# Priceincoding/nebula

Hardware: AMD Instinct MI355X
Metric: GTEPS for GO 3 STEPS on RMAT-26 at 1/2/4/8 GPUs; % of HBM roofline (higher is better)
Workload: dtype int64; 1 GPU; GO 3 STEPS FROM 64 seeds OVER follow WHERE follow.weight > 499 YIELD DISTINCT follow._dst; RMAT-26 ef16; vertices=32803048, edges_after_collapse=1060378721, edges_scanned_per_query=1545132647, parallelism=1 GPU

## Files before the change

### nebula_amd/csrc/bottom_up.hip

```cpp
#include <algorithm>
#include <cstdio>
#include <cstdlib>
#include <mutex>
#include <string>
#include <unordered_map>
#include <vector>

#include "device_common.h"
#include "engine.h"
#include "expr_device.h"
#include "go_device.h"
#include "go_launch.h"
#include "qpred.h"
#include "query_common.h"

namespace nbg {

__global__ __launch_bounds__(1024) void k_reduce_partials(const unsigned long long* partials, int nblocks,
                                                          unsigned long long* out,
                                                          const unsigned long long* gate = nullptr) {
  if (gate && *gate == 0ull) return;
  __shared__ unsigned long long s[kSlots][16];
  unsigned long long a[kSlots];
#pragma unroll
// ... 89 lines not shown
#pragma unroll
      for (int j = 0; j < R; j++) {
        const int64_t bj = __shfl((long long)rb[j], my_src), ej = __shfl((long long)re[j], my_src);
        if (my_j == j) {
          b = bj;
          e = ej;
        }
      }
      acc[3] += gl == 0 && my_j >= 0;
      bool f = false;
      for (int64_t x = b;; x += GL * ru) {
        const bool act = !f && x < e;
        if (__ballot(act) == 0) break;
        bool h = false;
        if (act) {
          int32_t sr[kRestMax];
#pragma unroll
          for (int u = 0; u < kRestMax; u++) {
            const int64_t ex = x + u * GL + gl;
            sr[u] = (u < ru && ex < e) ? tcol[ex] : -1;
          }
#pragma unroll
          for (int u = 0; u < kRestMax; u++) {
            const int64_t ex = x + u * GL + gl;
            if (sr[u] < 0) continue;
            acc[4]++;
            if (entry(sr[u], ex)) h = true;
          }
        }
        const unsigned long long hb = __ballot(h);
        if (act && ((hb >> (grp * GL)) & ((1ull << GL) - 1ull))) f = true;
      }
#pragma unroll
      for (int g = 0; g < NG; g++) {
        const int sj = __shfl(my_j, g * GL), ss = __shfl(my_src, g * GL);
        const int fg = __shfl(int(f), g * GL);
#pragma unroll
        for (int j = 0; j < R; j++)
          if (sj == j && lane == ss) found[j] = fg != 0;
      }
    }
  }
}

template <int PK, int U, int HUB, int STATS, int NT = 0, int SKIP = 0>
__global__ __launch_bounds__(1024, 8) void k_bu_lean(const uint2* __restrict__ lo, const uint2* __restrict__ hi,
                                                     int64_t ntiles, int64_t work_tiles,
                                                     const uint32_t* __restrict__ fbits, uint32_t fb_bytes,
                                                     unsigned long long* __restrict__ nbits,
                                                     unsigned long long* __restrict__ pbits,
                                                     const uint32_t* __restrict__ odeg, QArgs q_arg,
                                                     unsigned long long* __restrict__ partials, int cw,
                                                     const uint8_t* __restrict__ odeg8,
                                                     unsigned long long* gate, GateIn gi, int atomic_sums) {
  if (!gate_open(gi, gate)) return;
  __shared__ unsigned long long lds[kSlots * 16];
  extern __shared__ uint32_t s_fb[];
  if (HUB) hub_fill(s_fb, fbits, cw, true);
  const QArgs q = q_sgpr(q_arg);
  constexpr bool FINAL = PK == PK_FAST;
  constexpr int NS = FINAL ? 4 : 2;
  const __amdgpu_buffer_rsrc_t fb_rs =
      __builtin_amdgcn_make_buffer_rsrc(const_cast<uint32_t*>(fbits), 0, int(fb_bytes), 0x00020000);
  const uint32_t gmask = q.gmask, ucw = uint32_t(cw);
  const int lane = threadIdx.x & 63;
  const int64_t wave = (int64_t(blockIdx.x) * blockDim.x + threadIdx.x) >> 6;
  const int64_t nwaves = (int64_t(gridDim.x) * blockDim.x) >> 6;
  uint32_t nglob = 0, nhub = 0;
  unsigned long long nfound = 0, npend = 0, nwords = 0;
  unsigned long long odsum = 0;
  auto prep = [&](uint32_t sw, int k, uint32_t& goff, uint32_t& lidx, uint32_t& pm, uint32_t& um) {
    const uint32_t wi = (sw & gmask) >> 5;
    bool cand = true;
    if (FINAL) {
      const int st = q_test(int32_t(sw), q);
      const bool und = st < 0, pass = st > 0;
      cand = st != 0;
      pm |= pass ? 1u << k : 0u;
      um |= und ? 1u << k : 0u;
    }
    const bool hub = HUB && wi < ucw;
    goff = cand && !hub ? wi * 4u : 0xfffffff0u;
    lidx = cand && hub ? wi : ucw;
    if (STATS) {
      nglob += cand && !hub;
      nhub += cand && hub;
    }
  };
  auto bit = [](uint32_t w, uint32_t sw) -> uint32_t { return __builtin_amdgcn_ubfe(w, sw & 31u, 1u); };
  auto row_of = [&](int64_t t, int h) -> int64_t { return t * 128 + lane + 64 * h; };
  for (int64_t t0 = wave * U; t0 < work_tiles; t0 += nwaves * U) {
    uint2 a[U][2], b[U][2];
    uint32_t od[U][2];
    bool v[U];
#pragma unroll
    for (int u = 0; u < U; u++) {
      v[u] = t0 + u < work_tiles;
      const int64_t r = (v[u] ? t0 + u : t0) * 128 + lane;
#pragma unroll
      for (int h = 0; h < 2; h++) {
        if (NT) {
          const uint64_t x = __builtin_nontemporal_load(reinterpret_cast<const uint64_t*>(lo + r + 64 * h));
          a[u][h] = make_uint2(uint32_t(x), uint32_t(x >> 32));
          if (FINAL) {
            const uint64_t y = __builtin_nontemporal_load(reinterpret_cast<const uint64_t*>(hi + r + 64 * h));
            b[u][h] = make_uint2(uint32_t(y), uint32_t(y >> 32));
          }
          od[u][h] = FINAL ? 1u : uint32_t(__builtin_nontemporal_load(odeg8 + r + 64 * h));
        } else {
          a[u][h] = lo[r + 64 * h];
          if (FINAL) b[u][h] = hi[r + 64 * h];
          od[u][h] = FINAL ? 1u : odeg[r + 64 * h];
        }
      }
    }
    __builtin_amdgcn_sched_barrier(0);
    uint32_t goff[U][2][NS], lidx[U][2][NS], pm[U][2], um[U][2];
#pragma unroll
    for (int u = 0; u < U; u++)
#pragma unroll
      for (int h = 0; h < 2; h++) {
        pm[u][h] = um[u][h] = 0u;
        prep(a[u][h].x, 0, goff[u][h][0], lidx[u][h][0], pm[u][h], um[u][h]);
        prep(a[u][h].y, 1, goff[u][h][1], lidx[u][h][1], pm[u][h], um[u][h]);
        if (FINAL) {
          prep(b[u][h].x, 2, goff[u][h][2], lidx[u][h][2], pm[u][h], um[u][h]);
          prep(b[u][h].y, 3, goff[u][h][3], lidx[u][h][3], pm[u][h], um[u][h]);
        }
      }
    uint32_t lw[U][2][NS], gw[U][2][NS];
    if (HUB) {
#pragma unroll
      for (int u = 0; u < U; u++)
#pragma unroll
        for (int h = 0; h < 2; h++)
#pragma unroll
          for (int k = 0; k < NS; k++) {
            if (SKIP) {
              lw[u][h][k] = 0u;
              if (__ballot(lidx[u][h][k] != ucw)) lw[u][h][k] = s_fb[lidx[u][h][k]];
            } else {
              lw[u][h][k] = s_fb[lidx[u][h][k]];
            }
          }
    }
    bool noprobe[U][2];
#pragma unroll
    for (int u = 0; u < U; u++)
#pragma unroll
      for (int h = 0; h < 2; h++) {
        noprobe[u][h] = false;
        if ((SKIP & 2) && HUB && !FINAL) {
          const uint32_t sw[2] = {a[u][h].x, a[u][h].y};
          bool hf = false;
#pragma unroll
          for (int k = 0; k < NS; k++) hf = hf || bit(lw[u][h][k], sw[k]) != 0u;
          noprobe[u][h] = hf || od[u][h] == 0u;
        }
      }
#pragma unroll
    for (int u = 0; u < U; u++)
#pragma unroll
      for (int h = 0; h < 2; h++)
#pragma unroll
        for (int k = 0; k < NS; k++) {
          if (SKIP) {
            gw[u][h][k] = 0u;
            const uint32_t go = noprobe[u][h] ? 0xfffffff0u : goff[u][h][k];
            if (__ballot(go != 0xfffffff0u)) gw[u][h][k] = __builtin_amdgcn_raw_buffer_load_b32(fb_rs, go, 0, 0);
          } else {
            gw[u][h][k] = __builtin_amdgcn_raw_buffer_load_b32(fb_rs, goff[u][h][k], 0, 0);
          }
        }
    __builtin_amdgcn_sched_barrier(0);
    bool f[U][2], pend[U][2];
#pragma unroll
    for (int u = 0; u < U; u++) {
#pragma unroll
      for (int h = 0; h < 2; h++) {
        const uint32_t sw[4] = {a[u][h].x, a[u][h].y, b[u][h].x, b[u][h].y};
        uint32_t hm = 0u;
#pragma unroll
        for (int k = 0; k < NS; k++) hm |= bit(HUB ? (lw[u][h][k] | gw[u][h][k]) : gw[u][h][k], sw[k]) << k;
        if (FINAL) {
          f[u][h] = (hm & pm[u][h]) != 0u;
          pend[u][h] = v[u] && !f[u][h] && (b[u][h].y != 0xffffffffu || (hm & um[u][h]) != 0u);
        } else {
          f[u][h] = hm != 0u && od[u][h] > 0;
          pend[u][h] = v[u] && hm == 0u && od[u][h] > 0 && a[u][h].y != 0xffffffffu;
        }
      }
      nwords += v[u] ? (FINAL ? 8u : 4u) * 64u : 0u;
    }
    if (!FINAL) {
      bool anyp = false;
#pragma unroll
      for (int u = 0; u < U; u++) anyp = anyp || pend[u][0] || pend[u][1];
      const unsigned long long anyb = __ballot(anyp);
      if (anyb) {
#pragma unroll
        for (int u = 0; u < U; u++)
#pragma unroll
          for (int h = 0; h < 2; h++) {
            b[u][h] = make_uint2(0xffffffffu, 0xffffffffu);
            if (pend[u][h]) b[u][h] = hi[row_of(t0 + u, h)];
          }
        uint64_t pc = 0;
#pragma unroll
        for (int u = 0; u < U; u++) pc += uint64_t(__popcll(__ballot(pend[u][0])) + __popcll(__ballot(pend[u][1])));
        nwords += 2 * pc;
        uint32_t g2[U][2][2], l2[U][2][2];
#pragma unroll
        for (int u = 0; u < U; u++)
#pragma unroll
          for (int h = 0; h < 2; h++) {
            uint32_t d0 = 0u, d1 = 0u;
            prep(b[u][h].x, 0, g2[u][h][0], l2[u][h][0], d0, d1);
            prep(b[u][h].y, 1, g2[u][h][1], l2[u][h][1], d0, d1);
          }
        uint32_t lv[U][2][2], gv[U][2][2];
        if (HUB) {
#pragma unroll
          for (int u = 0; u < U; u++)
#pragma unroll
            for (int h = 0; h < 2; h++)
#pragma unroll
              for (int k = 0; k < 2; k++) lv[u][h][k] = s_fb[l2[u][h][k]];
        }
#pragma unroll
        for (int u = 0; u < U; u++)
#pragma unroll
          for (int h = 0; h < 2; h++)
#pragma unroll
            for (int k = 0; k < 2; k++) gv[u][h][k] = __builtin_amdgcn_raw_buffer_load_b32(fb_rs, g2[u][h][k], 0, 0);
#pragma unroll
        for (int u = 0; u < U; u++)
#pragma unroll
          for (int h = 0; h < 2; h++) {
            const uint32_t w0 = HUB ? (lv[u][h][0] | gv[u][h][0]) : gv[u][h][0];
            const uint32_t w1 = HUB ? (lv[u][h][1] | gv[u][h][1]) : gv[u][h][1];
            const bool g = (bit(w0, b[u][h].x) | bit(w1, b[u][h].y)) != 0u;
            f[u][h] = f[u][h] || (pend[u][h] && g);
            pend[u][h] = pend[u][h] && !g && b[u][h].y != 0xffffffffu;
          }
      } else {
#pragma unroll
        for (int u = 0; u < U; u++) pend[u][0] = pend[u][1] = false;
      }
    }
#pragma unroll
    for (int u = 0; u < U; u++) {
      if (!v[u]) continue;
      const int64_t t = t0 + u;
      unsigned long long f0 = __ballot(f[u][0]), f1 = __ballot(f[u][1]);
      unsigned long long p0 = __ballot(pend[u][0]), p1 = __ballot(pend[u][1]);
      if (SKIP & 4) {
        if (lane < 2) {
          typedef unsigned long long u64x2 __attribute__((ext_vector_type(2)));
          u64x2 vv;
          vv.x = lane ? p0 : f0;
          vv.y = lane ? p1 : f1;
          *reinterpret_cast<u64x2*>((lane ? pbits : nbits) + 2 * t) = vv;
        }
      } else if (lane < 2) {
        nbits[2 * t + lane] = lane ? f1 : f0;
        pbits[2 * t + lane] = lane ? p1 : p0;
      }
      nfound += uint64_t(__popcll(f0) + __popcll(f1));
      npend += uint64_t(__popcll(p0) + __popcll(p1));
      if (!FINAL) {
#pragma unroll
        for (int h = 0; h < 2; h++) {
          uint32_t d = f[u][h] ? od[u][h] : 0u;
          if (NT && d == 255u) d = odeg[row_of(t, h)];
          odsum += uint64_t(d);
        }
      }
    }
  }
  for (int64_t t = work_tiles + wave; t < ntiles; t += nwaves)
    if (lane < 2) {
      nbits[2 * t + lane] = 0ull;
      pbits[2 * t + lane] = 0ull;
    }
  if (lane != 0) nfound = npend = nwords = 0;
  unsigned long long acc64[8] = {nfound, odsum, nwords, npend, 0, 0, nglob, nhub};
  if (atomic_sums) block_add_sums(acc64, 8, lds, partials, atomic_sums);
  else block_store_partials(acc64, 8, lds, partials);
}

constexpr uint32_t kNoProbe = 0x0ffffff0u;
template <int CLS, int NT>
__global__ __launch_bounds__(1024, 8) void k_bu_fin(const uint2* __restrict__ lo, const uint2* __restrict__ hi,
                                                    int64_t ntiles, int64_t work_tiles,
                                                    const uint32_t* __restrict__ fbits,
                                                    unsigned long long* __restrict__ nbits,
                                                    unsigned long long* __restrict__ pbits, FinArgs fa_arg,
                                                    unsigned long long* __restrict__ partials, int cw,
                                                    uint32_t fb_rest, unsigned long long* gate, GateIn gi,
                                                    int atomic_sums, const uint32_t* __restrict__ wide) {
  if (!gate_open(gi, gate)) return;
  extern __shared__ uint32_t s_fb[];
  unsigned long long* lds = reinterpret_cast<unsigned long long*>(s_fb + ((cw + 2) & ~1));
  hub_fill(s_fb, fbits, cw, true);
  const uint32_t clo = __builtin_amdgcn_readfirstlane(fa_arg.clo), cr = __builtin_amdgcn_readfirstlane(fa_arg.cr);
  const uint32_t plo = __builtin_amdgcn_readfirstlane(fa_arg.plo), pr = __builtin_amdgcn_readfirstlane(fa_arg.pr);
  const bool pinv = __builtin_amdgcn_readfirstlane(fa_arg.pinv) != 0;
  const uint32_t bmask = __builtin_amdgcn_readfirstlane(fa_arg.bmask);
  const uint32_t cw4 = __builtin_amdgcn_readfirstlane(uint32_t(cw) * 4u);
  const __amdgpu_buffer_rsrc_t fb_rs = __builtin_amdgcn_make_buffer_rsrc(
      const_cast<uint32_t*>(fbits + cw), 0, int(__builtin_amdgcn_readfirstlane(fb_rest)), 0x00020000);
  typedef const __attribute__((address_space(3))) uint32_t* lds_u32p;
  const int lane = threadIdx.x & 63;
  const int64_t wave =
      int64_t(__builtin_amdgcn_readfirstlane(uint32_t((int64_t(blockIdx.x) * blockDim.x + threadIdx.x) >> 6)));
  const int64_t nwaves = (int64_t(gridDim.x) * blockDim.x) >> 6;
  unsigned long long nfound = 0, npend = 0, nwords = 0;
  auto ld8 = [&](const uint2* p) -> uint2 {
    if (!NT) return *p;
    const uint64_t x = __builtin_nontemporal_load(reinterpret_cast<const uint64_t*>(p));
    return make_uint2(uint32_t(x), uint32_t(x >> 32));
  };
  const uint32_t rest_b = __builtin_amdgcn_readfirstlane(fb_rest);
  auto tile = [&](int64_t t, auto ns_c) {
    constexpr int NS = decltype(ns_c)::value;
    uint32_t sw[2][NS];
    const int64_t r = t * 128 + lane;
#pragma unroll
    for (int h = 0; h < 2; h++) {
      const uint2 a = ld8(lo + r + 64 * h);
      sw[h][0] = a.x, sw[h][1] = a.y;
      if (NS == 4) {
        const uint2 b = ld8(hi + r + 64 * h);
        sw[h][NS - 2] = b.x, sw[h][NS - 1] = b.y;
      }
    }
    __builtin_amdgcn_sched_barrier(0);
    uint32_t ob[2][NS];
// ... 435 lines not shown
      c.opt("bu_atomic_sums", 1) != 0 && c.opt("bu_rest_dbg", 0) == 0 ? (out_zero ? std::max(shards, 1) : 1) : 0;
  p.ru = int(std::max<int64_t>(1, std::min<int64_t>(c.opt("bu_unroll", 1), kRestMax)));
  p.W = p.fast ? int(fp.width) : 0;
  p.rcw = int(std::min<int64_t>(c.opt(p.fast ? "bu_rest_lds_kb_final" : "bu_rest_lds_kb", 0) * 256,
                                std::min<int64_t>({fb_words, int64_t(36 * 1024), hub_cap})));
  p.rshm = size_t(std::max(p.rcw, 1)) * 4;
  p.rsteps = int(std::max<int64_t>(1, c.opt("bu_rest_steps", 4)));
  p.rest_rows = std::min(tr.n_rows, p.work * 128);
  p.use_rec = es.brec.p && es.brec_rows >= std::min(tr.n_rows, p.work * 128) && c.opt("bu_rec", 1) != 0;
  return p;
}

struct BuOut {
  unsigned long long* nb;
  unsigned long long* pbits;
  unsigned long long* partials;
  unsigned long long* gate;
};

void bu_first_pass(Ctx& c, const EdgeSpace& es, const BuPlan& p, const uint32_t* fb, const uint32_t* odeg,
                   const BuOut& o, const GateIn& gi, BuLaunch& L) {
  const uint2* lo = es.pair_col[0].as<uint2>();
  const uint2* hi = es.pair_col[1].as<uint2>();
  const int cw = p.cw;
  if (p.fast && !p.probe_stats && c.opt("bu_fin", 1) != 0) {
    using Fn = decltype(&k_bu_fin<0, 0>);
    static const Named<Fn> fin[4] = {NBG_K(k_bu_fin<0, 0>), NBG_K(k_bu_fin<1, 0>), NBG_K(k_bu_fin<0, 1>),
                                     NBG_K(k_bu_fin<1, 1>)};
    const FinArgs fa = fin_args(p.q);
    const bool cls1 = fin_cls1_ok(fa) && c.opt("bu_fin_cls", 1) != 0;
    const size_t fshm = size_t((cw + 2) & ~1) * 4 + size_t(kSlots) * 16 * 8;
    const uint32_t rest = p.fb_bytes > uint32_t(cw) * 4u ? p.fb_bytes - uint32_t(cw) * 4u : 0u;
    const int nt = int(c.opt("bu_fin_nt", 1) != 0);
    const uint32_t* wide = c.opt("bu_fin_narrow", 1) != 0 ? es.tile_wide.as<uint32_t>() : nullptr;
    if (wide) L.flag_bytes = uint64_t(p.work) / 8;
    const Named<Fn>& k = fin[(cls1 ? 1 : 0) | nt << 1];
    if (fshm > 48 * 1024) lds_limit(reinterpret_cast<const void*>(k.fn), fshm);
    k.fn<<<p.grid, p.bs, fshm, c.stream>>>(lo, hi, p.ntiles, p.work, fb, o.nb, o.pbits, fa, o.partials, cw, rest, o.gate,
                                           gi, p.atomic_sums, wide);
    L.k0 = k.name;
    return;
  }
  enum { kPlain, kHub, kPlainStats, kHubStats, kHubNt };
  using Fn = decltype(&k_bu_lean<0, 1, 0, 0, 0, 0>);
  static const Named<Fn> lean[2][5] = {
      {NBG_K(k_bu_lean<0, 1, 0, 0, 0, 0>), NBG_K(k_bu_lean<0, 1, 1, 0, 0, 0>), NBG_K(k_bu_lean<0, 1, 0, 1, 0, 0>),
       NBG_K(k_bu_lean<0, 1, 1, 1, 0, 0>), NBG_K(k_bu_lean<0, 1, 1, 0, 1, 3>)},
      {NBG_K(k_bu_lean<1, 1, 0, 0, 0, 0>), NBG_K(k_bu_lean<1, 1, 1, 0, 0, 0>), NBG_K(k_bu_lean<1, 1, 0, 1, 0, 0>),
       NBG_K(k_bu_lean<1, 1, 1, 1, 0, 0>), NBG_K(k_bu_lean<1, 1, 1, 0, 1, 3>)}};
  int sel = p.probe_stats ? (cw > 0 ? kHubStats : kPlainStats) : (cw > 0 ? kHub : kPlain);
  if (sel == kHub && (p.fast || es.odeg8.p)) sel = kHubNt;
  const Named<Fn>& k = lean[p.pk][sel];
  if (p.shm > 48 * 1024) lds_limit(reinterpret_cast<const void*>(k.fn), p.shm);
  k.fn<<<p.grid, p.bs, p.shm, c.stream>>>(lo, hi, p.ntiles, p.work, fb, p.fb_bytes, o.nb, o.pbits,
                                          p.fast ? nullptr : odeg, p.q, o.partials, cw, es.odeg8.as<uint8_t>(), o.gate,
                                          gi, p.atomic_sums);
  L.k0 = k.name;
  if (!p.fast) L.od_bytes = uint64_t(p.work) * 128u * (sel == kHubNt ? 1u : 4u);
}

void bu_rest_pass(Ctx& c, const EdgeSpace& es, const BuPlan& p, const uint32_t* fb, const uint32_t* odeg,
                  const FastArgs& fp, const BuOut& o, unsigned long long* dbg, BuLaunch& L) {
  using Fn = decltype(&k_bu_rest_lean<0, 0, 0, 0>);
#define NBG_REST_ROW(PKV, WV)                                                                     \
  {NBG_K(k_bu_rest_lean<PKV, WV, 0, 0>), NBG_K(k_bu_rest_lean<PKV, WV, 0, 1>), \
   NBG_K(k_bu_rest_lean<PKV, WV, 1, 0>), NBG_K(k_bu_rest_lean<PKV, WV, 1, 1>)}
  static const Named<Fn> rest_none[4] = NBG_REST_ROW(0, 0);
  static const Named<Fn> rest_fast[4][4] = {NBG_REST_ROW(1, 1), NBG_REST_ROW(1, 2), NBG_REST_ROW(1, 4),
                                            NBG_REST_ROW(1, 8)};
#undef NBG_REST_ROW
  const int wi = p.W == 1 ? 0 : p.W == 2 ? 1 : p.W == 4 ? 2 : 3;
  const Named<Fn>& k = (p.fast ? rest_fast[wi] : rest_none)[(p.rcw > 0 ? 2 : 0) | (p.use_rec ? 1 : 0)];
  const Csr& tr = es.tr;
  const int32_t* tc = p.q.gbits ? es.tcol_q.as<int32_t>() : tr.col.as<int32_t>();
  const uint4* rec = p.use_rec ? es.brec.as<uint4>() : nullptr;
  if (p.rshm > 48 * 1024) lds_limit(reinterpret_cast<const void*>(k.fn), p.rshm);
  k.fn<<<p.grid2, 1024, p.rshm, c.stream>>>(o.pbits, p.rest_rows, tr.row_ptr.as<int64_t>(), tc, fb, p.fb_bytes, o.nb,
                                            odeg, fp, p.q, p.atomic_sums ? o.partials : o.partials + p.grid, p.rcw, p.ru,
                                            p.rest_from, p.rsteps, dbg, o.gate, rec, p.atomic_sums);
  L.k1 = k.name;
  L.rest_rec = p.use_rec;
}
#undef NBG_K

void bu_rest_dbg_dump(Ctx& c, const unsigned long long* dbg, int pk, int grid2) {
  std::vector<unsigned long long> h(size_t(grid2) * 16 * 8);
  NBG_HIP(hipMemcpyAsync(h.data(), dbg, h.size() * 8, hipMemcpyDeviceToHost, c.stream));
  NBG_HIP(hipStreamSynchronize(c.stream));
  if (const char* fn = getenv("NBG_DBG_FILE")) {
    if (FILE* f = fopen(fn, "ab")) {
      const uint64_t hdr[2] = {uint64_t(pk), uint64_t(grid2) * 16};
      fwrite(hdr, 8, 2, f);
      fwrite(h.data(), 8, h.size(), f);
      fclose(f);
    }
  }
}

}

BuLaunch launch_bu_lean(Ctx& c, EdgeSpace& es, const uint32_t* fb, uint32_t* nbits, const uint32_t* odeg, int pk,
                        const FastArgs& fp, int fcol, unsigned long long* out, bool hop_front, unsigned long long* gate,
                        GateIn gi, bool out_zero, int shards) {
  const BuPlan p = bu_plan(c, es, pk, !odeg, fp, fcol, hop_front, out_zero, shards);
  c.ws_pend.ensure(size_t(p.ntiles * 2 + 2) * 8);
  const BuOut o{reinterpret_cast<unsigned long long*>(nbits), c.ws_pend.as<unsigned long long>(),
                p.atomic_sums ? out : c.ws_partials.as<unsigned long long>(), gate};
  if (p.atomic_sums && !out_zero) NBG_HIP(hipMemsetAsync(out, 0, 8 * 8, c.stream));
  BuLaunch L;
  bu_first_pass(c, es, p, fb, odeg, o, gi, L);
  NBG_HIP(hipGetLastError());
// ... 25 lines not shown
```

### nebula_amd/csrc/csr_build.hip

```cpp
#include <climits>

#include <rocprim/device/device_merge.hpp>
#include <rocprim/device/device_reduce.hpp>
#include <rocprim/device/device_scan.hpp>

#include "build_common.h"
#include "qpred.h"

namespace nbg {

__global__ void k_iota_rev_u32(uint32_t* p, int64_t n) {
  for (int64_t i = blockIdx.x * int64_t(blockDim.x) + threadIdx.x; i < n; i += int64_t(gridDim.x) * blockDim.x)
    p[i] = uint32_t(n - 1 - i);
}
__global__ void k_iota_u32(uint32_t* p, int64_t n) {
  for (int64_t i = blockIdx.x * int64_t(blockDim.x) + threadIdx.x; i < n; i += int64_t(gridDim.x) * blockDim.x)
    p[i] = uint32_t(i);
}
__global__ void k_edge_keys(const int64_t* src, const int64_t* dst, int64_t n, const int64_t* keys_ht,
                            const int32_t* vals_ht, uint64_t mask, bool has_min, int32_t min_gidx,
                            int64_t lo, int64_t hi, const uint32_t* byterank, uint64_t* keys,
                            uint32_t* perm, int32_t* dst_g, unsigned long long* err) {
  for (int64_t i = blockIdx.x * int64_t(blockDim.x) + threadIdx.x; i < n; i += int64_t(gridDim.x) * blockDim.x) {
    int32_t sg = ht_lookup(keys_ht, vals_ht, mask, src[i], has_min, min_gidx);
// ... 594 lines not shown
  }
  if (maxd) atomicMax(maxd, m);
}
__global__ void k_hub_key(const int32_t* tsrc, int64_t m, const uint32_t* gdeg, uint32_t maxd, uint32_t* key) {
  for (int64_t i = blockIdx.x * int64_t(blockDim.x) + threadIdx.x; i < m; i += int64_t(gridDim.x) * blockDim.x)
    key[i] = maxd - gdeg[tsrc[i]];
}
__global__ void k_minmax_w(const void* data, int w, int64_t m, long long* mm) {
  long long lo = LLONG_MAX, hi = LLONG_MIN;
  for (int64_t i = blockIdx.x * int64_t(blockDim.x) + threadIdx.x; i < m; i += int64_t(gridDim.x) * blockDim.x) {
    long long v = w == 1 ? static_cast<const int8_t*>(data)[i]
                : w == 2 ? static_cast<const int16_t*>(data)[i]
                : w == 4 ? static_cast<const int32_t*>(data)[i]
                         : static_cast<const int64_t*>(data)[i];
    lo = v < lo ? v : lo;
    hi = v > hi ? v : hi;
  }
  for (int o = 32; o > 0; o >>= 1) {
    const long long a = __shfl_xor(lo, o), b = __shfl_xor(hi, o);
    lo = a < lo ? a : lo;
    hi = b > hi ? b : hi;
  }
  if ((threadIdx.x & 63) == 0) {
    atomicMin(mm, lo);
    atomicMax(mm + 1, hi);
  }
}
__global__ void k_pack_col(const int32_t* col, const void* data, int w, int64_t m, int64_t vmin, uint64_t range,
                           int gbits, int qbits, int32_t* out) {
  for (int64_t i = blockIdx.x * int64_t(blockDim.x) + threadIdx.x; i < m; i += int64_t(gridDim.x) * blockDim.x) {
    const int64_t v = w == 1 ? static_cast<const int8_t*>(data)[i]
                    : w == 2 ? static_cast<const int16_t*>(data)[i]
                    : w == 4 ? static_cast<const int32_t*>(data)[i]
                             : static_cast<const int64_t*>(data)[i];
    out[i] = int32_t((q_bucket(v, vmin, range, qbits) << gbits) | uint32_t(col[i]));
  }
}
template <typename T>
__global__ void k_build_pair(const int64_t* trp, const T* src, int64_t n, T* lo, T* hi, T none) {
  for (int64_t d = blockIdx.x * int64_t(blockDim.x) + threadIdx.x; d < n; d += int64_t(gridDim.x) * blockDim.x) {
    const int64_t b = trp[d], e = trp[d + 1];
#pragma unroll
    for (int q = 0; q < 4; q++) (q < 2 ? lo : hi)[size_t(d) * 2 + (q & 1)] = b + q < e ? src[b + q] : none;
  }
}

__global__ void k_tile_wide(const int64_t* trp, int64_t n, uint32_t* wide) {
  const int lane = threadIdx.x & 63;
  for (int64_t b = blockIdx.x * int64_t(blockDim.x) + threadIdx.x - lane; b < n; b += int64_t(gridDim.x) * blockDim.x) {
    const int64_t d = b + lane;
    const bool w = d < n && trp[d + 1] - trp[d] >= 3;
    const int64_t t = b >> 7;
    if (__ballot(w) != 0ull && lane == 0) atomicOr(wide + (t >> 5), 1u << (uint32_t(t) & 31u));
  }
}

__global__ void k_build_rec(const int64_t* trp, const int32_t* src, int64_t n, uint4* rec) {
  for (int64_t d = blockIdx.x * int64_t(blockDim.x) + threadIdx.x; d < n; d += int64_t(gridDim.x) * blockDim.x) {
    const int64_t b = trp[d], e = trp[d + 1];
    const uint64_t deg = uint64_t(e - b) < 65535u ? uint64_t(e - b) : 65535u;
    uint32_t w[16];
    w[0] = uint32_t(uint64_t(b));
    w[1] = uint32_t(uint64_t(b) >> 32) | uint32_t(deg << 16);
#pragma unroll
    for (int k = 0; k < kRecEntries; k++) w[2 + k] = b + k < e ? uint32_t(src[b + k]) : 0xffffffffu;
#pragma unroll
    for (int j = 0; j < 4; j++) rec[size_t(d) * 4 + j] = make_uint4(w[4 * j], w[4 * j + 1], w[4 * j + 2], w[4 * j + 3]);
  }
}

std::array<long long, 2> minmax_w(Ctx& c, const void* data, int width, int64_t n) {
  DevWords<long long, 2> mm;
  mm.set(c, {LLONG_MAX, LLONG_MIN});
  if (n) k_minmax_w<<<grid_for(n), 256, 0, c.stream>>>(data, width, n, mm.dev());
  return mm.read(c);
}

void build_out_degrees(Ctx& c, EdgeSpace& es, const uint8_t* row_ok, unsigned int* dmax) {
  const int64_t n = es.out.n_rows, n_pad = (n + 127) / 128 * 128;
  es.odeg.alloc(size_t(n_pad + 1) * 4);
  NBG_HIP(hipMemsetAsync(es.odeg.p, 0, size_t(n_pad + 1) * 4, c.stream));
  k_out_deg<<<grid_for(n), 256, 0, c.stream>>>(es.out.row_ptr.as<int64_t>(), row_ok, n, es.odeg.as<uint32_t>(), dmax);
}

void row_part_by_hash(Ctx& c, const int64_t* vids, int64_t n, int32_t* row_part) {
  k_row_part_default<<<grid_for(n), 256, 0, c.stream>>>(vids, n, c.num_parts, row_part);
}

struct TransposeBuild {
  Ctx& c;
  EdgeSpace& es;
  Csr& o;
  Csr& t;
  const int64_t m, lo, n_own;
  const int G;
  DevBuf gdeg;
  const uint32_t* gdegp = nullptr;
  uint32_t maxd = 0;
  DevBuf tdst, tsrc;
  int64_t R = 0;
  std::vector<const PropCol*> cp;
  std::vector<DevBuf> rprops;
  std::vector<const void*> psrc;
  DevBuf perm;

  TransposeBuild(Ctx& ctx, EdgeSpace& e)
// ... 141 lines not shown
      t.props[f].data.alloc(size_t(R) * size_t(w) + 16);
      if (R) gather_width(c, psrc[f], perm.as<uint32_t>(), t.props[f].data.p, R, w);
      rprops[f].release();
    }
    if (G == 1) {
      es.t_eid = std::move(perm);
      es.has_t_eid = true;
    } else {
      es.has_t_eid = false;
    }
  }

  void pack_quantised() {
    es.q_field = -1;
    es.q_gbits = es.q_bits = 0;
    es.tcol_q.release();
    if (R <= 0) return;
    const int gb = bits_for(c.n_global + 1);
    const int qb = std::min(8, 31 - gb);
    int f = -1;
    for (size_t i = 0; i < t.props.size() && f < 0; i++)
      if (t.props[i].data.p) f = int(i);
    if (qb < 3 || f < 0) return;
    const PropCol& pc = t.props[size_t(f)];
    const auto h = minmax_w(c, pc.data.p, pc.width, R);
    es.q_field = f;
    es.q_gbits = gb;
    es.q_bits = qb;
    es.q_min = h[0];
    es.q_range = uint64_t(h[1]) - uint64_t(h[0]) + 1;
    es.tcol_q.alloc(size_t(R) * 4 + 64);
    k_pack_col<<<grid_for(R), 256, 0, c.stream>>>(t.col.as<int32_t>(), pc.data.p, pc.width, R, es.q_min, es.q_range, gb,
                                                  qb, es.tcol_q.as<int32_t>());
    NBG_HIP(hipGetLastError());
  }
  const int32_t* first_pass_col() const { return es.q_field >= 0 ? es.tcol_q.as<int32_t>() : t.col.as<int32_t>(); }

  void pair_slab() {
    const int64_t n_pad = (n_own + 127) / 128 * 128;
    for (int h = 0; h < 2; h++) {
      es.pair_col[h].alloc(size_t(n_pad) * 8 + 16);
      NBG_HIP(hipMemsetAsync(es.pair_col[h].as<uint8_t>() + size_t(n_own) * 8, 0xff, size_t(n_pad - n_own) * 8 + 16,
                             c.stream));
    }
    if (n_own)
      k_build_pair<int32_t><<<grid_for(n_own), 256, 0, c.stream>>>(t.row_ptr.as<int64_t>(), first_pass_col(), n_own,
                                                                   es.pair_col[0].as<int32_t>(),
                                                                   es.pair_col[1].as<int32_t>(), -1);
    const int64_t nt = n_pad / 128;
    es.tile_wide.alloc(size_t(nt / 32 + 2) * 4);
    NBG_HIP(hipMemsetAsync(es.tile_wide.p, 0, size_t(nt / 32 + 2) * 4, c.stream));
    if (n_own)
      k_tile_wide<<<grid_for(n_own), 256, 0, c.stream>>>(t.row_ptr.as<int64_t>(), n_own, es.tile_wide.as<uint32_t>());
  }
  void live_bounds() {
    DevWords<unsigned long long, 2> lb;
    lb.zero(c);
    if (n_own)
      k_live_bounds<<<grid_for(n_own), 256, 0, c.stream>>>(t.row_ptr.as<int64_t>(), es.odeg.as<uint32_t>(), n_own,
                                                           lb.dev());
    const auto h = lb.read(c);
    es.bu_in_tiles = int64_t((h[0] + 127) / 128);
    es.bu_both_tiles = int64_t((h[1] + 127) / 128);
  }
  void rest_records() {
    es.brec.release();
    es.brec_rows = 0;
    const int64_t rows = std::min(n_own, es.bu_in_tiles * 128);
    const int64_t cap_mb = c.opt("bu_rec_mb", 8192);
    if (rows > 0 && c.opt("bu_rec", 1) != 0 && rows * 64 <= (cap_mb << 20)) {
      es.brec.alloc(size_t(rows) * 64);
      k_build_rec<<<grid_for(rows), 256, 0, c.stream>>>(t.row_ptr.as<int64_t>(), first_pass_col(), rows,
                                                        es.brec.as<uint4>());
      NBG_HIP(hipGetLastError());
      es.brec_rows = rows;
    }
  }
};

void build_transpose(Ctx& c, EdgeSpace& es) {
  TransposeBuild b(c, es);
  b.out_degrees();
  if (b.G == 1) b.transposed_edges_local();
  else b.transposed_edges_exchange();
  b.hub_first_order();
  for (int h = 0; h < 2; h++) es.pair_col[h].release();
  es.tile_wide.release();
  b.pack_quantised();
  b.pair_slab();
  b.live_bounds();
  b.rest_records();
  NBG_HIP(hipStreamSynchronize(c.stream));
  NBG_HIP(hipGetLastError());
  es.has_tr = true;
}

}
```

### nebula_amd/csrc/engine.h

```cpp
#pragma once
#include <hip/hip_runtime.h>

#include <atomic>
#include <chrono>
#include <cstdint>
#include <cstdio>
#include <cstring>
#include <map>
#include <memory>
#include <mutex>
#include <stdexcept>
#include <string>
#include <vector>

#include "../../include/nebula_amd.h"

namespace nbg {

struct Error : std::runtime_error {
  int32_t code;
  Error(int32_t c, const std::string& m) : std::runtime_error(m), code(c) {}
};

#define NBG_HIP(x)                                                                        \
// ... 243 lines not shown
  DevBuf ov_prop_table;
  size_t bytes() const {
    size_t b = row_ptr.bytes + col.bytes + col_vid.bytes + rank.bytes + row_part.bytes + row_ok.bytes + ov_edge.bytes;
    for (auto& p : props) b += p.data.bytes + p.present.bytes + p.str_off.bytes + p.str_bytes.bytes;
    for (auto& p : ov_props) b += p.data.bytes + p.present.bytes + p.str_off.bytes + p.str_bytes.bytes;
    return b;
  }
};

struct Staging {
  int64_t n = 0;
  DevBuf src, dst, rank, ver;
  DevBuf part;
  DevBuf seq;
  bool rank_const = true, ver_const = true;
  int64_t rank_value = 0, ver_value = 0;
  std::vector<DevBuf> props;
  std::vector<DevBuf> present;
  std::vector<DevBuf> str_len;
  size_t cap = 0;
};

struct EdgeSpace {
  int32_t type = 0;
  int32_t schema_ver = 0;
  std::vector<Field> fields;
  Staging out_stage, in_stage;
  Csr out, in;
  Csr rep_out, rep_in;
  bool has_rep = false, has_rep_out = false;
  DevBuf rep_odeg;
  Csr tr;
  DevBuf t_eid;
  bool has_tr = false;
  bool has_t_eid = false;
  int64_t out_nnz_global = -1;
  struct Order {
    DevBuf perm, skey, dstg;
    int64_t n = 0;
  };
  Order ord[2];
  bool rmat_stream = false;
  int32_t rmat_scale = 0, rmat_ef = 0;
  uint64_t rmat_seed = 0;
  DevBuf odeg;
  int64_t max_odeg = -1;
  int64_t max_odeg_global = -1;
  std::vector<int64_t> top_deg;
  int64_t bu_in_tiles = 0;
  int64_t bu_both_tiles = 0;
  DevBuf odeg8;
  DevBuf pair_col[2];
  DevBuf tile_wide;
  int32_t q_field = -1, q_gbits = 0, q_bits = 0;
  int64_t q_min = 0;
  uint64_t q_range = 1;
  DevBuf tcol_q;
  DevBuf brec;
  int64_t brec_rows = 0;
  struct Rev {
    bool built = false;
    DevBuf ideg;
    int64_t max_ideg_global = -1;
    std::vector<int64_t> top_deg;
    int64_t in_nnz_global = -1;
    int mirror = -1;
  } rev;
  bool kv_loaded = false;
};
constexpr int kRecEntries = 14;

struct TagSpace {
  int32_t id = 0;
  int32_t schema_ver = 0;
  std::string name;
  std::vector<Field> fields;
  Staging stage;
  int64_t committed_n = 0;
  std::vector<PropCol> cols;
  DevBuf part;
  int64_t n_tail = 0;
  DevBuf tail_vids;
  DevBuf state;
};
struct TagFieldRef {
  std::string tag, prop;
  int32_t type;
};

struct Timing {
  double total_ms = 0, expand_ms = 0;
  int64_t expand_launches = 0;
  uint64_t edges_scanned = 0, expand_bytes = 0;
  int32_t steps_run = 0;
  int32_t bu_steps = 0;
  double comm_ms = 0;
  uint64_t comm_bytes = 0;
  int32_t n_hops = 0;
  nbg_hop_stat hops[NBG_MAX_HOP_STATS] = {};
  int32_t host_waits = 0;
  int32_t spec_hops = 0;
  int32_t launches = 0;
  int32_t comm_calls = 0;
  uint64_t hop_bytes_mark = 0;
  void hop(int32_t mode, bool final_hop, double ms, const unsigned long long* c6, double kernel_ms = -1,
           uint64_t kernel_bytes = 0) {
    const uint64_t b = expand_bytes - hop_bytes_mark;
    hop_bytes_mark = expand_bytes;
    if (n_hops >= NBG_MAX_HOP_STATS) return;
    nbg_hop_stat& h = hops[n_hops++];
    h.mode = mode;
    h.final_hop = final_hop ? 1 : 0;
    h.ms = ms;
    h.bytes = b;
    for (int i = 0; i < 8; i++) h.c[i] = c6 ? c6[i] : 0;
    h.kernel_ms = kernel_ms < 0 ? ms : kernel_ms;
    h.kernel_bytes = kernel_ms < 0 ? b : kernel_bytes;
  }
  void name_last_hop(const std::string& k0, const std::string& k1 = "", const char* k2 = nullptr) {
    if (n_hops == 0 || n_hops > NBG_MAX_HOP_STATS) return;
    std::string s = k0;
    if (!k1.empty()) s += "; " + k1;
    if (k2) s += std::string("; ") + k2;
// ... 211 lines not shown
```

### nebula_amd/csrc/snapshot.hip

```cpp
#include <algorithm>
#include <numeric>

#include "build_common.h"

namespace nbg {

constexpr int kMaxFields = 64;
struct SchemaDev {
  int32_t nfields;
  int32_t types[kMaxFields];
};

static std::shared_ptr<BufPool> build_pool(Ctx& c) {
  const int64_t gb = c.opt("build_pool_gb", 128);
  if (gb <= 0) return nullptr;
  c.build_pool->limit = size_t(gb) << 30;
  return c.build_pool;
}

__global__ void k_hash_part(const int64_t* src, int32_t* part, int64_t n, int32_t parts) {
  for (int64_t i = blockIdx.x * int64_t(blockDim.x) + threadIdx.x; i < n; i += int64_t(gridDim.x) * blockDim.x)
    part[i] = int32_t(uint64_t(src[i]) % uint64_t(parts) + 1);
}

// ... 339 lines not shown
  }
  for (auto& kvp : c.tags) {
    TagSpace& ts = kvp.second;
    size_t nf = ts.fields.size();
    SchemaDev sch{};
    sch.nfields = int32_t(nf);
    for (size_t f = 0; f < nf; f++) sch.types[f] = ts.fields[f].type;
    stage_reserve(c, ts.stage, nf, n, true, ts.fields);
    NBG_HIP(hipMemsetAsync(cnt.p, 0, 64, c.stream));
    unsigned long long* d = cnt.as<unsigned long long>();
    NBG_HIP(hipMemcpyAsync(d, &ts.stage.n, 8, hipMemcpyHostToDevice, c.stream));
    k_decode_vkv<<<grid_for(int64_t(n)), 256, 0, c.stream>>>(
        dk.as<uint8_t>(), dko.as<uint64_t>(), c.heap.as<uint8_t>() + heap_base, dvo.as<uint64_t>(), int64_t(n),
        ts.id, ts.schema_ver, sch, heap_base, c.load_seq, stage_ptrs(ts.stage, nf), d, d + 2, part);
    NBG_HIP(hipGetLastError());
    unsigned long long h[5];
    NBG_HIP(hipMemcpyAsync(h, d, 40, hipMemcpyDeviceToHost, c.stream));
    NBG_HIP(hipStreamSynchronize(c.stream));
    ts.stage.n = int64_t(h[0]);
    if (h[3] != 0) throw Error(NBG_E_UNSUPPORTED, "tag row schema version differs from the registered version");
    if (h[4] != 0) throw Error(NBG_E_PART_NOT_FOUND, "vertex key of another part");
  }
  } catch (...) {
    for (auto& m : marks) m.s->n = m.n;
    c.heap_used = heap_mark;
    c.load_seq += int64_t(n);
    throw;
  }
  c.load_seq += int64_t(n);
  c.build_seconds += now_s() - t0;
}

void snapshot_load_part(Ctx& c, int32_t part, const uint8_t* kb, const uint64_t* koff,
                        const uint8_t* vb, const uint64_t* voff, size_t n) {
  PoolScope build_scope(build_pool(c));
  if (c.finalized) throw Error(NBG_E_STATE, "snapshot already finalized");
  decode_part(c, part, kb, koff, vb, voff, n);
}

static void reset_transpose_derived(EdgeSpace& es) {
  es.rep_out = Csr();
  es.rep_in = Csr();
  es.has_rep = es.has_rep_out = false;
  es.rep_odeg.release();
  es.tr = Csr();
  es.t_eid.release();
  es.has_tr = es.has_t_eid = false;
  es.out_nnz_global = -1;
  es.tcol_q.release();
  es.q_field = -1;
  es.q_gbits = es.q_bits = 0;
  for (int h = 0; h < 2; h++) es.pair_col[h].release();
  es.tile_wide.release();
  es.odeg.release();
  es.odeg8.release();
  es.max_odeg = -1;
  es.max_odeg_global = -1;
  es.top_deg.clear();
  es.bu_in_tiles = es.bu_both_tiles = 0;
  es.brec.release();
  es.brec_rows = 0;
  es.rev = EdgeSpace::Rev();
}

static void reset_edge_derived(EdgeSpace& es) {
  es.out = Csr();
  es.in = Csr();
  reset_transpose_derived(es);
}

static void reset_derived(Ctx& c) {
  c.brank.release();
  for (auto& kv : c.edges)
    for (auto& o : kv.second.ord) {
      o.perm.release();
      o.skey.release();
      o.dstg.release();
      o.n = 0;
    }
  c.vid_of.release();
  c.ht_keys.release();
  c.ht_vals.release();
  c.ht_cap = 0;
  c.ht_has_min = false;
  c.ht_min_gidx = -1;
  c.tag_table.release();
  for (auto& kv : c.edges) reset_edge_derived(kv.second);
  for (auto& kv : c.tags) {
    kv.second.cols.clear();
    kv.second.part.release();
  }
  c.sp_dist[0].release();
  c.sp_dist[1].release();
  c.sp_dist_bytes = 0;
  c.sp_dirty = false;
  c.sp = Ctx::SpWork();
}

static bool commit_merge(Ctx& c);

void snapshot_write_part(Ctx& c, int32_t part, const uint8_t* kb, const uint64_t* koff,
                         const uint8_t* vb, const uint64_t* voff, size_t n) {
  PoolScope build_scope(build_pool(c));
  if (!c.finalized) {
    decode_part(c, part, kb, koff, vb, voff, n);
    return;
// ... 989 lines not shown
```

Before: 4134 GTEPS.

## Add per-tile shape summary to skip out-degree loads and hi-column pending checks

Builds a per-128-row tile shape word at transpose build time, recording whether any row in the tile has three or more in-edges and whether all active rows share one out-degree. The bottom-up lean kernel reads this word per tile, prefetched one iteration ahead through a scalar register. For uniform-degree tiles it skips the per-row out-degree load and computes the degree sum as popcount times the degree. For tiles with no wide rows it suppresses pending marks, so no hi-column follow-up is needed. This aims to cut HBM traffic on the odeg arrays and reduce rest-pass work, at the cost of an extra build kernel, a small shape array, and more scalar logic in the hot loop.

New measurement: 4241 GTEPS, median of 6. 2.6% higher.

```diff
diff --git a/nebula_amd/csrc/bottom_up.hip b/nebula_amd/csrc/bottom_up.hip
--- a/nebula_amd/csrc/bottom_up.hip
+++ b/nebula_amd/csrc/bottom_up.hip
@@ -165,7 +165,8 @@
                                                      const uint32_t* __restrict__ odeg, QArgs q_arg,
                                                      unsigned long long* __restrict__ partials, int cw,
                                                      const uint8_t* __restrict__ odeg8,
-                                                     unsigned long long* gate, GateIn gi, int atomic_sums) {
+                                                     unsigned long long* gate, GateIn gi, int atomic_sums,
+                                                     const uint32_t* __restrict__ shape, int tile_stats) {
   if (!gate_open(gi, gate)) return;
   __shared__ unsigned long long lds[kSlots * 16];
   extern __shared__ uint32_t s_fb[];
@@ -182,6 +183,14 @@
   uint32_t nglob = 0, nhub = 0;
   unsigned long long nfound = 0, npend = 0, nwords = 0;
   unsigned long long odsum = 0;
+  unsigned long long odsum_u = 0;
+  auto shape_index = [&](int64_t t) -> uint32_t {
+    return __builtin_amdgcn_readfirstlane(uint32_t(min(t, work_tiles)));
+  };
+  auto shape_word = [&](uint32_t i) -> uint32_t { return FINAL || !shape ? kShapeWide | kShapeMixed : shape[i]; };
+  uint32_t shn[U];
+#pragma unroll
+  for (int u = 0; u < U; u++) shn[u] = shape_word(shape_index(wave * U + u));
   auto prep = [&](uint32_t sw, int k, uint32_t& goff, uint32_t& lidx, uint32_t& pm, uint32_t& um) {
     const uint32_t wi = (sw & gmask) >> 5;
     bool cand = true;
@@ -195,7 +204,7 @@
     const bool hub = HUB && wi < ucw;
     goff = cand && !hub ? wi * 4u : 0xfffffff0u;
     lidx = cand && hub ? wi : ucw;
-    if (STATS) {
+    if (STATS && !tile_stats) {
       nglob += cand && !hub;
       nhub += cand && hub;
     }
@@ -206,6 +215,21 @@
     uint2 a[U][2], b[U][2];
     uint32_t od[U][2];
     bool v[U];
+    bool two[U], uni[U];
+    uint32_t ud[U];
+#pragma unroll
+    for (int u = 0; u < U; u++) {
+      uint32_t cur = shn[u];
+      if (!FINAL) {
+        uint32_t ni = shape_index(t0 + nwaves * U + u);
+        asm volatile("" : "+s"(cur), "+s"(ni));
+        __builtin_amdgcn_sched_barrier(0);
+        shn[u] = shape_word(ni);
+      }
+      two[u] = (cur & kShapeWide) == 0u;
+      ud[u] = cur & kShapeMixed;
+      uni[u] = ud[u] != kShapeMixed;
+    }
 #pragma unroll
     for (int u = 0; u < U; u++) {
       v[u] = t0 + u < work_tiles;
@@ -219,11 +243,13 @@
             const uint64_t y = __builtin_nontemporal_load(reinterpret_cast<const uint64_t*>(hi + r + 64 * h));
             b[u][h] = make_uint2(uint32_t(y), uint32_t(y >> 32));
           }
-          od[u][h] = FINAL ? 1u : uint32_t(__builtin_nontemporal_load(odeg8 + r + 64 * h));
+          od[u][h] = FINAL ? 1u : ud[u];
+          if (!FINAL && !uni[u]) od[u][h] = uint32_t(__builtin_nontemporal_load(odeg8 + r + 64 * h));
         } else {
           a[u][h] = lo[r + 64 * h];
           if (FINAL) b[u][h] = hi[r + 64 * h];
-          od[u][h] = FINAL ? 1u : odeg[r + 64 * h];
+          od[u][h] = FINAL ? 1u : ud[u];
+          if (!FINAL && !uni[u]) od[u][h] = odeg[r + 64 * h];
         }
       }
     }
@@ -300,7 +326,7 @@
           pend[u][h] = v[u] && !f[u][h] && (b[u][h].y != 0xffffffffu || (hm & um[u][h]) != 0u);
         } else {
           f[u][h] = hm != 0u && od[u][h] > 0;
-          pend[u][h] = v[u] && hm == 0u && od[u][h] > 0 && a[u][h].y != 0xffffffffu;
+          pend[u][h] = v[u] && !two[u] && hm == 0u && od[u][h] > 0 && a[u][h].y != 0xffffffffu;
         }
       }
       nwords += v[u] ? (FINAL ? 8u : 4u) * 64u : 0u;
@@ -382,11 +408,21 @@
       nfound += uint64_t(__popcll(f0) + __popcll(f1));
       npend += uint64_t(__popcll(p0) + __popcll(p1));
       if (!FINAL) {
-#pragma unroll
-        for (int h = 0; h < 2; h++) {
-          uint32_t d = f[u][h] ? od[u][h] : 0u;
-          if (NT && d == 255u) d = odeg[row_of(t, h)];
-          odsum += uint64_t(d);
+        if (uni[u]) {
+          odsum_u += uint64_t(ud[u]) * uint64_t(__popcll(f0) + __popcll(f1));
+        } else {
+#pragma unroll
+          for (int h = 0; h < 2; h++) {
+            uint32_t d = f[u][h] ? od[u][h] : 0u;
+            if (NT && d == 255u) d = odeg[row_of(t, h)];
+            odsum += uint64_t(d);
+          }
+        }
+        if (STATS && tile_stats) {
+          const bool c6 = tile_stats == 2 ? two[u] && uni[u] : two[u];
+          const bool c7 = tile_stats == 2 ? !two[u] && !uni[u] : uni[u];
+          nglob += lane == 0 && c6;
+          nhub += lane == 0 && c7;
         }
       }
     }
@@ -397,6 +433,7 @@
       pbits[2 * t + lane] = 0ull;
     }
   if (lane != 0) nfound = npend = nwords = 0;
+  if (lane == 0) odsum += odsum_u;
   unsigned long long acc64[8] = {nfound, odsum, nwords, npend, 0, 0, nglob, nhub};
   if (atomic_sums) block_add_sums(acc64, 8, lds, partials, atomic_sums);
   else block_store_partials(acc64, 8, lds, partials);
@@ -938,11 +975,17 @@
   if (sel == kHub && (p.fast || es.odeg8.p)) sel = kHubNt;
   const Named<Fn>& k = lean[p.pk][sel];
   if (p.shm > 48 * 1024) lds_limit(reinterpret_cast<const void*>(k.fn), p.shm);
+  const uint32_t* shape = !p.fast && odeg == es.odeg.as<uint32_t>() && c.opt("bu_lean_shape", 1) != 0
+                              ? es.tile_shape.as<uint32_t>()
+                              : nullptr;
   k.fn<<<p.grid, p.bs, p.shm, c.stream>>>(lo, hi, p.ntiles, p.work, fb, p.fb_bytes, o.nb, o.pbits,
                                           p.fast ? nullptr : odeg, p.q, o.partials, cw, es.odeg8.as<uint8_t>(), o.gate,
-                                          gi, p.atomic_sums);
+                                          gi, p.atomic_sums, shape, p.probe_stats > 1 ? p.probe_stats - 1 : 0);
   L.k0 = k.name;
-  if (!p.fast) L.od_bytes = uint64_t(p.work) * 128u * (sel == kHubNt ? 1u : 4u);
+  if (!p.fast) {
+    const uint64_t od_tiles = shape ? uint64_t(p.work - std::min(p.work, es.shape_tiles[0])) : uint64_t(p.work);
+    L.od_bytes = od_tiles * 128u * (sel == kHubNt ? 1u : 4u) + (shape ? uint64_t(p.work) * 4u : 0u);
+  }
 }
 
 void bu_rest_pass(Ctx& c, const EdgeSpace& es, const BuPlan& p, const uint32_t* fb, const uint32_t* odeg,
diff --git a/nebula_amd/csrc/csr_build.hip b/nebula_amd/csrc/csr_build.hip
--- a/nebula_amd/csrc/csr_build.hip
+++ b/nebula_amd/csrc/csr_build.hip
@@ -670,6 +670,43 @@
     const bool w = d < n && trp[d + 1] - trp[d] >= 3;
     const int64_t t = b >> 7;
     if (__ballot(w) != 0ull && lane == 0) atomicOr(wide + (t >> 5), 1u << (uint32_t(t) & 31u));
+  }
+}
+
+__global__ void k_tile_shape(const int64_t* trp, const uint32_t* odeg, int64_t n, int64_t ntiles, uint32_t* shape) {
+  const int lane = threadIdx.x & 63;
+  const int64_t wave = (blockIdx.x * int64_t(blockDim.x) + threadIdx.x) >> 6;
+  const int64_t nwaves = (int64_t(gridDim.x) * blockDim.x) >> 6;
+  for (int64_t t = wave; t < ntiles; t += nwaves) {
+    bool wide = false, has[2];
+    uint32_t o[2];
+#pragma unroll
+    for (int h = 0; h < 2; h++) {
+      const int64_t d = t * 128 + lane + 64 * h;
+      const int64_t ind = d < n ? trp[d + 1] - trp[d] : 0;
+      wide = wide || ind >= 3;
+      has[h] = ind > 0;
+      o[h] = has[h] ? odeg[d] : 0u;
+    }
+    const unsigned long long b0 = __ballot(has[0]), b1 = __ballot(has[1]);
+    uint32_t d0 = kShapeMixed;
+    if (b0) d0 = uint32_t(__shfl(int(o[0]), __ffsll((long long)b0) - 1));
+    else if (b1) d0 = uint32_t(__shfl(int(o[1]), __ffsll((long long)b1) - 1));
+    const bool mixed = (has[0] && o[0] != d0) || (has[1] && o[1] != d0);
+    const bool w = __ballot(wide) != 0ull, m = __ballot(mixed) != 0ull || d0 >= kShapeMixed;
+    if (lane == 0) shape[t] = (w ? kShapeWide : 0u) | (m ? kShapeMixed : d0);
+  }
+}
+__global__ void k_shape_count(const uint32_t* shape, int64_t nt, unsigned long long* out) {
+  unsigned long long a[4] = {0, 0, 0, 0};
+  for (int64_t t = blockIdx.x * int64_t(blockDim.x) + threadIdx.x; t < nt; t += int64_t(gridDim.x) * blockDim.x) {
+    const uint32_t s = shape[t];
+    const bool uni = (s & kShapeMixed) != kShapeMixed, two = !(s & kShapeWide);
+    a[0] += uni, a[1] += two, a[2] += uni && two, a[3] += (s & kShapeMixed) == 0u;
+  }
+  for (int k = 0; k < 4; k++) {
+    for (int o = 32; o > 0; o >>= 1) a[k] += (unsigned long long)__shfl_xor((long long)a[k], o);
+    if ((threadIdx.x & 63) == 0 && a[k]) atomicAdd(out + k, a[k]);
   }
 }
 
@@ -917,6 +954,24 @@
     NBG_HIP(hipMemsetAsync(es.tile_wide.p, 0, size_t(nt / 32 + 2) * 4, c.stream));
     if (n_own)
       k_tile_wide<<<grid_for(n_own), 256, 0, c.stream>>>(t.row_ptr.as<int64_t>(), n_own, es.tile_wide.as<uint32_t>());
+    es.tile_shape.alloc(size_t(nt + 2) * 4);
+    NBG_HIP(hipMemsetAsync(es.tile_shape.p, 0xff, size_t(nt + 2) * 4, c.stream));
+    if (n_own)
+      k_tile_shape<<<grid_for(nt * 64), 256, 0, c.stream>>>(t.row_ptr.as<int64_t>(), es.odeg.as<uint32_t>(), n_own, nt,
+                                                           es.tile_shape.as<uint32_t>());
+  }
+  void shape_shares() {
+    DevWords<unsigned long long, 4> sc;
+    sc.zero(c);
+    if (es.bu_both_tiles > 0)
+      k_shape_count<<<grid_for(es.bu_both_tiles), 256, 0, c.stream>>>(es.tile_shape.as<uint32_t>(), es.bu_both_tiles,
+                                                                      sc.dev());
+    const auto h = sc.read(c);
+    for (int k = 0; k < 3; k++) es.shape_tiles[k] = int64_t(h[size_t(k)]);
+    if (h[3]) {
+      es.tile_shape.release();
+      es.shape_tiles[0] = es.shape_tiles[1] = es.shape_tiles[2] = 0;
+    }
   }
   void live_bounds() {
     DevWords<unsigned long long, 2> lb;
@@ -951,9 +1006,11 @@
   b.hub_first_order();
   for (int h = 0; h < 2; h++) es.pair_col[h].release();
   es.tile_wide.release();
+  es.tile_shape.release();
   b.pack_quantised();
   b.pair_slab();
   b.live_bounds();
+  b.shape_shares();
   b.rest_records();
   NBG_HIP(hipStreamSynchronize(c.stream));
   NBG_HIP(hipGetLastError());
diff --git a/nebula_amd/csrc/engine.h b/nebula_amd/csrc/engine.h
--- a/nebula_amd/csrc/engine.h
+++ b/nebula_amd/csrc/engine.h
@@ -319,6 +319,8 @@
   DevBuf odeg8;
   DevBuf pair_col[2];
   DevBuf tile_wide;
+  DevBuf tile_shape;
+  int64_t shape_tiles[3] = {0, 0, 0};
   int32_t q_field = -1, q_gbits = 0, q_bits = 0;
   int64_t q_min = 0;
   uint64_t q_range = 1;
@@ -336,6 +338,7 @@
   bool kv_loaded = false;
 };
 constexpr int kRecEntries = 14;
+constexpr uint32_t kShapeWide = 0x80000000u, kShapeMixed = 0x7fffffffu;
 
 struct TagSpace {
   int32_t id = 0;
diff --git a/nebula_amd/csrc/snapshot.hip b/nebula_amd/csrc/snapshot.hip
--- a/nebula_amd/csrc/snapshot.hip
+++ b/nebula_amd/csrc/snapshot.hip
@@ -415,6 +415,7 @@
   es.q_gbits = es.q_bits = 0;
   for (int h = 0; h < 2; h++) es.pair_col[h].release();
   es.tile_wide.release();
+  es.tile_shape.release();
   es.odeg.release();
   es.odeg8.release();
   es.max_odeg = -1;
```
